# oriolfornes/ExplaiNN

Hardware: AMD Instinct MI355X
Metric: sequences/sec (fwd+bwd), 200bp one-hot, 300 units, batch 1024 (higher is better)
Workload: dtype f32

## Files before the change

explainn_amd/csrc/api.hip:

```cpp
#include <stdarg.h>
#include <stdio.h>
#include <string.h>

#include <cstdlib>
#include <cstring>

#include "common.h"

static thread_local char g_err[512] = "";

void explainn_set_error(const char* fmt, ...) {
    va_list ap;
    va_start(ap, fmt);
    vsnprintf(g_err, sizeof(g_err), fmt, ap);
    va_end(ap);
}

extern "C" const char* explainn_last_error(void) { return g_err; }

namespace {
struct Carver {
    int64_t off = 0;
    char* base = nullptr;
    template <typename T>
    void take(T** p, int64_t count) {
        off = (off + 255) & ~int64_t(255);
        if (base) *p = reinterpret_cast<T*>(base + off);
        off += count * (int64_t)sizeof(T);
    }
};

void carve(explainn_ctx* c, Carver& cv) {
    const int64_t U = c->U, U4 = c->U4, n = c->n, Bs = c->Bs, NS = c->NS, K4 = c->K4;
    cv.take(&c->codesT, (int64_t)c->L * Bs);
    cv.take(&c->pk2, (int64_t)c->PW * Bs);
    cv.take(&c->nmask, (int64_t)c->NW * Bs);
    cv.take(&c->bm, (int64_t)4 * (Bs / 64) * c->Lp);
    cv.take(&c->G, K4 * K4);
    cv.take(&c->m, K4);
    cv.take(&c->alpha, U4);
    cv.take(&c->shift, U4);
    cv.take(&c->mug, U4);
    cv.take(&c->sig1, U4);
    cv.take(&c->Gw, U4 * K4);
    cv.take(&c->Wt, (int64_t)c->Uq * c->k * 20);
    cv.take(&c->Wf, (int64_t)conv_tiles_padded(c->U, c->k) * conv_ksteps(c->k) * 3 * 512);
    cv.take(&c->Wsg, (int64_t)conv_tiles_padded(c->U, c->k) * 32);
    const int64_t Upad = (int64_t)32 * conv_tiles_padded(c->U, c->k);
    cv.take(&c->ext, Upad * n * Bs + 64);
    cv.take(&c->idx, Upad * n * Bs + 64);
    cv.take(&c->qs0, U * NS);
    cv.take(&c->qS1p, U * c->QCH * NS);
    cv.take(&c->qS2p, U * c->QCH * NS * NS);
    cv.take(&c->qbar, U * NS);
    cv.take(&c->VC, U * FC_H * NS);
    cv.take(&c->A2, U * FC_H * NS);
    cv.take(&c->A2f, c->NQ <= FC_BF_MAXN ? 0 : U * FC_MT * fc_nk4q(c->NQ) * 256);
    cv.take(&c->A2h, c->NQ <= FC_BF_MAXN ? U * FC_MT * fc_ks32(c->NQ) * 3 * 256 : 0);
    cv.take(&c->sh2, U * FC_H);
    cv.take(&c->sig2, U * FC_H);
    cv.take(&c->z, U * Bs);
    cv.take(&c->zhat, U * Bs);
    cv.take(&c->o, U * Bs);
    cv.take(&c->sig3, U);
    c->ZBLK = fc_fwd_blocks((int)Bs, c->NQ);
    cv.take(&c->z12p, U * c->ZBLK * 2);
    cv.take(&c->bits, U * Bs + 4);
    cv.take(&c->dz, U * Bs + 4);
    cv.take(&c->EQp, U * c->ACH * FC_H * NS);
    cv.take(&c->Sep, U * c->ACH * FC_H);
    cv.take(&c->EQs, U * FC_H * NS);
    cv.take(&c->Ttf, U * fc_nw16(c->NQ) * 3 * 4 * 256);
    cv.take(&c->Mff, U * fc_nw16(c->NQ) * 4 * fc_nw16(c->NQ) * 64);
    cv.take(&c->k0p, U * NS);
    cv.take(&c->dy, U4 * n * Bs);
    cv.take(&c->S12p, U * fc_ng(c->NQ) * (Bs / 16) * 2);
    cv.take(&c->Dspp, U * (Bs / 4) * K4);
    cv.take(&c->dlogits, (int64_t)c->maxB * c->T);
    cv.take(&c->flags, 64);
    cv.take(&c->dlT, (int64_t)c->T * Bs);
    cv.take(&c->gWp, c->T > HEAD_GEMM_MIN_T ? (int64_t)head_gw_chunks(c->maxB) * c->T * (c->U + 1) : 0);
    cv.take(&c->lossp, 256);
    cv.take(&c->site_cnt, U4 * Bs);
    cv.take(&c->site_off, U4 * Bs);
    cv.off = (cv.off + 255) & ~int64_t(255);
}

int check_batch(const explainn_ctx* c, int B) {
    if (!c) { explainn_set_error("null context"); return EXPLAINN_E_ARG; }
    if (B < 1 || B > c->maxB) {
        explainn_set_error("batch %d outside [1, max_batch=%d]", B, c->maxB);
        return EXPLAINN_E_ARG;
    }
    return EXPLAINN_OK;
}

#define TRY(call)                    \
    do {                             \
        int rc_ = (call);            \
        if (rc_ != EXPLAINN_OK) return rc_; \
    } while (0)

const char* const kStageNames[ST_COUNT] = {
    "pack_tables", "moments", "prep1_stats", "conv_pool", "qmom", "prep2", "fc_fwd", "head_fwd",
    "loss", "head_bwd", "passA", "mid", "passB", "conv_bwd", "fin_bwd"};
#define STAGE(id, call)                                                                 \
    do {                                                                                \
        if (c->timing) HIP_TRY(hipEventRecord(c->ev0[id], s));                          \
        TRY(call);                                                                      \
        if (c->timing) { HIP_TRY(hipEventRecord(c->ev1[id], s)); c->timed |= 1u << (id); } \
    } while (0)

int eval_front(explainn_ctx* c, const float* x, int B, const explainn_params* p, hipStream_t s) {
    c->fwd_B = 0; c->tail_B = 0;
    if (c->dense) {
        if (!x) { explainn_set_error("dense input mode needs x"); return EXPLAINN_E_ARG; }
        c->staged_B = 0;
    } else {
        TRY(launch_pack(c, x, B, false, s));
    }
    if (!(c->eval_valid && p->version != 0 && p->version == c->eval_version)) {
        TRY(launch_prep1_tables(c, p, s));
        TRY(launch_prep1(c, p, B, false, s));
        TRY(launch_prep2(c, p, B, false, s));
        c->eval_valid = true;
        c->eval_version = p->version;
// ... 408 lines not shown
```

explainn_amd/csrc/bwd.hip:

```cpp
#include "common.h"

typedef float f32x16b __attribute__((ext_vector_type(16)));
typedef float f32x2 __attribute__((ext_vector_type(2)));
typedef float f32x4b __attribute__((ext_vector_type(4)));

__global__ __launch_bounds__(1024) void mid_fused_kernel(
    const float* __restrict__ EQp, const float* __restrict__ Sep, const float* __restrict__ A2,
    const float* __restrict__ sh2, const float* __restrict__ sig2, const float* __restrict__ fc1_w,
    const float* __restrict__ fc2_w, const float* __restrict__ g2, const double* __restrict__ qbar,
    const float* __restrict__ VC, float* __restrict__ Ttf,
    float* __restrict__ Mff, float* __restrict__ k0p, float* __restrict__ g_fc2_w, float* __restrict__ g_bn2_w,
    float* __restrict__ g_bn2_b, float* __restrict__ g_fc1_b, float* __restrict__ g_fc1_w, int n,
    int NS, int NW16, int B, int ACH, float scale) {
    extern __shared__ float fsm[];
    const int ld = n + 1;
    float* V1s = fsm;
    float* A2s = V1s + FC_H * ld;
    float* EQl = A2s + FC_H * ld;
    float* Ms = EQl + FC_H * ld;
    float* qb = Ms + n * n;
    float* se = qb + n;
    float* md2s = se + FC_H;
    float* cfs = md2s + FC_H;
    float* md2hs = cfs + FC_H;
    float* VCl = md2hs + FC_H;
    float* svl = VCl + FC_H * ld;
    float* gsl = svl + FC_H;
    float* sgl = gsl + FC_H;
    const int u = blockIdx.x, tid = threadIdx.x;
    STAMP(0);
    {
        constexpr int NPASS = 3;
        for (int e0 = tid; e0 < FC_H * n; e0 += 1024 * NPASS) {
            float v1[NPASS], a2[NPASS], vc[NPASS];
            int dst[NPASS];
#pragma unroll
            for (int it = 0; it < NPASS; ++it) {
                const int e = e0 + 1024 * it;
                const bool on = e < FC_H * n;
                const int ec = on ? e : 0, r = ec / n, w = ec - r * n;
                const uint32_t ch = (uint32_t)(u * FC_H + r);
                dst[it] = on ? r * ld + w : -1;
                v1[it] = fc1_w[(size_t)ch * n + w];
                a2[it] = A2[(size_t)ch * NS + w];
                vc[it] = VC[(size_t)ch * NS + w];
            }
#pragma unroll
            for (int it = 0; it < NPASS; ++it) { KEEP(v1[it]); KEEP(a2[it]); KEEP(vc[it]); }
#pragma unroll
            for (int it = 0; it < NPASS; ++it)
                if (dst[it] >= 0) { V1s[dst[it]] = v1[it]; A2s[dst[it]] = a2[it]; VCl[dst[it]] = vc[it]; }
        }
    }
    for (int e0 = tid; e0 < FC_H * n; e0 += 1024 * 3) {
        double eq[3] = {0, 0, 0};
        for (int c0 = 0; c0 < ACH; c0 += 4) {
            float pv[3][4];
#pragma unroll
            for (int it = 0; it < 3; ++it) {
                const int e = e0 + 1024 * it, ec = e < FC_H * n ? e : 0;
                const int w = ec / FC_H, r = ec % FC_H;
#pragma unroll
                for (int i = 0; i < 4; ++i)
                    pv[it][i] = EQp[(((size_t)u * ACH + min(c0 + i, ACH - 1)) * NS + w) * FC_H + r];
// ... 31 lines not shown
    __syncthreads();
    STAMP(1);
    const double sc = (double)scale;
    if (tid < FC_H) {
        const int r = tid;
        const size_t ch = (size_t)u * FC_H + r;
        double sAE = 0, sVE = 0;
        const double ser = (double)se[r];
        for (int w = 0; w < n; ++w) {
            const double eq = (double)EQl[r * ld + w];
            sAE = fma((double)A2s[r * ld + w], eq, sAE);
            sVE = fma((double)V1s[r * ld + w], eq - ser * qbd[w], sVE);
        }
        const double v2 = (double)fc2_w[ch], sg = (double)sig2[ch];
        g_fc2_w[ch] = (float)(sc * (sAE + (double)sh2[ch] * ser));
        const double db2 = sc * v2 * ser, dg2 = sc * v2 / sg * sVE;
        g_bn2_b[ch] = (float)db2;
        g_bn2_w[ch] = (float)dg2;
        g_fc1_b[ch] = 0.f;
        md2s[r] = (float)(db2 / (double)B);
        md2hs[r] = (float)(dg2 / (double)B);
        cfs[r] = (float)((dg2 / (double)B) / sg);
        svl[r] = (float)v2; gsl[r] = (float)((double)g2[ch] / sg); sgl[r] = (float)((double)B / sg);
    }
    __syncthreads();
    STAMP(2);
    const int NT2 = NW16;
    const int ntile_m = NT2 * NT2;
    {
        const int wave = tid >> 6, lane = tid & 63, c = lane & 15, gq = lane >> 4;
        for (int tile = wave; tile < ntile_m; tile += 16) {
            const int vt = tile / NT2, wt = tile % NT2;
            const int va = 16 * vt + c, wb = 16 * wt + c;
            const bool alive = va < n, blive = wb < n;
            const float* acol = V1s + min(va, n - 1);
            const float* bcol = A2s + min(wb, n - 1);
            f32x4b acc = f32x4b{0.f, 0.f, 0.f, 0.f};
#pragma unroll
            for (int q0 = 0; q0 < FC_H / 4; q0 += 5) {
                float av[5], bv[5];
#pragma unroll
                for (int q = 0; q < 5; ++q) {
                    const int r = 4 * (q0 + q) + gq;
                    av[q] = cfs[r] * acol[r * ld];
                    bv[q] = bcol[r * ld];
                }
#pragma unroll
                for (int q = 0; q < 5; ++q)
                    acc = __builtin_amdgcn_mfma_f32_16x16x4f32(alive ? av[q] : 0.f, blive ? bv[q] : 0.f, acc, 0, 0, 0);
            }
#pragma unroll
            for (int i = 0; i < 4; ++i) {
                const int v = 16 * vt + 4 * gq + i;
                Mff[(((size_t)u * NW16 + wt) * (4 * NW16) + 4 * vt + i) * 64 + 16 * gq + c] = acc[i];
                if (v < n && wb < n) Ms[v * n + wb] = acc[i];
            }
        }
    }
    STAMP(3);
    const int busy = min(ntile_m, 8) * 64;
    for (int e = tid - busy; e < FC_H * NS; e += 1024 - busy) {
        if (e < 0) break;
        const int r = e / NS, w = e % NS;
        const size_t ch = (size_t)u * FC_H + r;
        const double sv = sc * (double)svl[r];
        float tv = 0.f;
        if (w < n) {
            tv = (float)(sv * (double)A2s[r * ld + w]);
            const double hq = (double)VCl[r * ld + w] * (double)sgl[r];
            const double val = (double)gsl[r] *
                               (sv * (double)EQl[r * ld + w] -
                                (double)md2s[r] * (double)B * qbd[w] -
                                (double)md2hs[r] * hq);
            g_fc1_w[ch * n + w] = (float)val;
        }
        {
            const uint32_t hb = __float_as_uint(tv) & 0xffff0000u;
            const float r1 = tv - __uint_as_float(hb);
            const uint32_t mb = __float_as_uint(r1) & 0xffff0000u;
            const float r2 = r1 - __uint_as_float(mb);
            uint16_t* tb = reinterpret_cast<uint16_t*>(Ttf) + ((size_t)u * NW16 + (w >> 4)) * (3 * 4 * 512) +
                           ((size_t)(r >> 5) * 64 + 16 * ((r >> 3) & 3) + (w & 15)) * 8 + (r & 7);
            tb[0] = (uint16_t)(hb >> 16);
            tb[4 * 512] = (uint16_t)(mb >> 16);
            tb[8 * 512] = (uint16_t)(__float_as_uint(r2) >> 16);
        }
    }
    __syncthreads();
    STAMP(4);
    for (int w = tid; w < NS; w += 1024) {
        double k0 = 0;
        if (w < n) {
            for (int r = 0; r < FC_H; ++r) k0 = fma((double)A2s[r * ld + w], (double)md2s[r], k0);
            for (int v = 0; v < n; ++v) k0 -= qbd[v] * (double)Ms[v * n + w];
        }
        k0p[(size_t)u * NS + w] = (float)k0;
    }
    STAMP(5);
}

__global__ __launch_bounds__(1024) void mid_big_kernel(
    const float* __restrict__ EQp, const float* __restrict__ Sep, const float* __restrict__ A2,
    const float* __restrict__ sh2, const float* __restrict__ sig2, const float* __restrict__ fc1_w,
    const float* __restrict__ fc2_w, const float* __restrict__ g2, const double* __restrict__ qbar,
    const float* __restrict__ VC, float* __restrict__ EQs,
    float* __restrict__ Ttf, float* __restrict__ Mff,
    float* __restrict__ k0p, float* __restrict__ g_fc2_w, float* __restrict__ g_bn2_w,
    float* __restrict__ g_bn2_b, float* __restrict__ g_fc1_b, float* __restrict__ g_fc1_w, int n,
    int NS, int NW16, int B, int ACH, float scale) {
    extern __shared__ float bsm[];
    const int ld = n + 1;
    float* V1s = bsm;
    float* A2s = V1s + FC_H * ld;
    float* qb = A2s + FC_H * ld;
    float* se = qb + n;
    float* md2s = se + FC_H;
    float* cfs = md2s + FC_H;
    float* md2hs = cfs + FC_H;
    float* kco = md2hs + FC_H;
    const int u = blockIdx.x, tid = threadIdx.x;
    constexpr int NT = 1024;
    for (int e = tid; e < FC_H * n; e += NT) {
        const int r = e / n, w = e % n;
        const size_t ch = (size_t)u * FC_H + r;
        V1s[r * ld + w] = fc1_w[ch * n + w];
        A2s[r * ld + w] = A2[ch * NS + w];
    }
    for (int e = tid; e < FC_H * n; e += NT) {
        const int w = e / FC_H, r = e % FC_H;
        const size_t ch = (size_t)u * FC_H + r;
        double eq = 0;
        for (int c0 = 0; c0 < ACH; c0 += 8) {
            float pv[8];
#pragma unroll
            for (int i = 0; i < 8; ++i)
                pv[i] = EQp[(((size_t)u * ACH + min(c0 + i, ACH - 1)) * NS + w) * FC_H + r];
#pragma unroll
            for (int i = 0; i < 8; ++i) KEEP(pv[i]);
#pragma unroll
            for (int i = 0; i < 8; ++i) eq += (c0 + i < ACH) ? (double)pv[i] : 0.0;
        }
        EQs[ch * NS + w] = (float)eq;
    }
    for (int w = tid; w < n; w += NT) qb[w] = (float)qbar[(size_t)u * NS + w];
    for (int r = tid; r < FC_H; r += NT) {
        double s = 0;
        for (int c = 0; c < ACH; ++c) s += (double)Sep[((size_t)u * ACH + c) * FC_H + r];
        se[r] = (float)s;
    }
    __syncthreads();
    const double sc = (double)scale;
    {
        const int r = tid >> 3, part = tid & 7;
        const int rr = r < FC_H ? r : FC_H - 1;
        const size_t ch = (size_t)u * FC_H + rr;
        double sAE = 0, sVE = 0, qv = 0;
        const double ser = (double)se[rr];
        for (int w = part; w < n; w += 8) {
            const double eq = (double)EQs[ch * NS + w];
            const double qw = qbar[(size_t)u * NS + w];
            sAE = fma((double)A2s[rr * ld + w], eq, sAE);
            sVE = fma((double)V1s[rr * ld + w], eq - ser * qw, sVE);
            qv = fma((double)V1s[rr * ld + w], qw, qv);
        }
#pragma unroll
        for (int off = 1; off < 8; off <<= 1) {
            sAE += __shfl_xor(sAE, off, 64); sVE += __shfl_xor(sVE, off, 64); qv += __shfl_xor(qv, off, 64);
        }
        if (r < FC_H && part == 0) {
            const double v2 = (double)fc2_w[ch], sg = (double)sig2[ch];
            g_fc2_w[ch] = (float)(sc * (sAE + (double)sh2[ch] * ser));
            const double db2 = sc * v2 * ser, dg2 = sc * v2 / sg * sVE;
            g_bn2_b[ch] = (float)db2;
            g_bn2_w[ch] = (float)dg2;
            g_fc1_b[ch] = 0.f;
            md2s[r] = (float)(db2 / (double)B);
            md2hs[r] = (float)(dg2 / (double)B);
            const double cf = (dg2 / (double)B) / sg;
            cfs[r] = (float)cf;
            kco[r] = (float)(db2 / (double)B - cf * qv);
        }
    }
    __syncthreads();
    {
        const int wave = tid >> 6, lane = tid & 63, rc = lane & 31, kk = lane >> 5;
        const int NT2 = (NS + 31) >> 5;
        for (int tile = wave; tile < NT2 * NT2; tile += NT / 64) {
            const int vt = tile / NT2, wt = tile % NT2;
            const int va = 32 * vt + rc, wb = 32 * wt + rc;
            const bool alive = va < n, blive = wb < n;
            const float* acol = V1s + min(va, n - 1);
            const float* bcol = A2s + min(wb, n - 1);
            f32x16b acc;
#pragma unroll
            for (int g = 0; g < 16; ++g) acc[g] = 0.f;
#pragma unroll 5
            for (int s2 = 0; s2 < FC_H / 2; ++s2) {
                const int r = 2 * s2 + kk;
                const float a = alive ? cfs[r] * acol[r * ld] : 0.f;
                const float bb = blive ? bcol[r * ld] : 0.f;
                acc = __builtin_amdgcn_mfma_f32_32x32x2f32(a, bb, acc, 0, 0, 0);
            }
            if (wb < NS) {
#pragma unroll
                for (int g = 0; g < 16; ++g) {
                    const int v = 32 * vt + (g & 3) + 8 * (g >> 2) + 4 * kk;
                    if (v < NS) {
                        if (v < 16 * NW16 && wb < 16 * NW16)
                            Mff[(((size_t)u * NW16 + (wb >> 4)) * (4 * NW16) + 4 * (v >> 4) + (v & 3)) * 64 +
                                16 * ((v >> 2) & 3) + (wb & 15)] = acc[g];
                    }
                }
            }
        }
    }
    for (int e = tid; e < FC_H * NS; e += NT) {
        const int r = e / NS, w = e % NS;
        const size_t ch = (size_t)u * FC_H + r;
        const double sv = sc * (double)fc2_w[ch];
        float tv = 0.f;
        if (w < n) {
            tv = (float)(sv * (double)A2s[r * ld + w]);
            const double sg = (double)sig2[ch];
            const double hq = (double)VC[ch * NS + w] * (double)B / sg;
            const double val = ((double)g2[ch] / sg) *
                               (sv * (double)EQs[ch * NS + w] -
                                (double)md2s[r] * (double)B * qbar[(size_t)u * NS + w] -
                                (double)md2hs[r] * hq);
            g_fc1_w[ch * n + w] = (float)val;
        }
        {
            const uint32_t hb = __float_as_uint(tv) & 0xffff0000u;
            const float r1 = tv - __uint_as_float(hb);
            const uint32_t mb = __float_as_uint(r1) & 0xffff0000u;
            const float r2 = r1 - __uint_as_float(mb);
            uint16_t* tb = reinterpret_cast<uint16_t*>(Ttf) + ((size_t)u * NW16 + (w >> 4)) * (3 * 4 * 512) +
                           ((size_t)(r >> 5) * 64 + 16 * ((r >> 3) & 3) + (w & 15)) * 8 + (r & 7);
            tb[0] = (uint16_t)(hb >> 16);
            tb[4 * 512] = (uint16_t)(mb >> 16);
            tb[8 * 512] = (uint16_t)(__float_as_uint(r2) >> 16);
        }
    }
    for (int w = tid; w < NS; w += NT) {
        double k0 = 0;
        if (w < n)
            for (int r = 0; r < FC_H; ++r) k0 = fma((double)A2s[r * ld + w], (double)kco[r], k0);
        k0p[(size_t)u * NS + w] = (float)k0;
    }
}

static size_t mid_big_lds(int n) {
    return ((size_t)2 * FC_H * (n + 1) + n + 5 * FC_H) * sizeof(float);
}

static size_t mid_fused_lds(int n) {
    return ((size_t)4 * FC_H * (n + 1) + (size_t)n * n + n + 7 * FC_H + 2) * sizeof(float) + (size_t)n * sizeof(double);
}

int launch_mid_bwd(explainn_ctx* c, const explainn_params* p, const explainn_grads* g, int B,
                   hipStream_t s) {
    if (c->n <= 72) {
        hipLaunchKernelGGL(mid_fused_kernel, dim3(c->U), dim3(1024), mid_fused_lds(c->n), s, c->EQp,
                           c->Sep, c->A2, c->sh2, c->sig2, p->fc1_w, p->fc2_w, p->bn2_w, c->qbar,
                           c->VC, c->Ttf, c->Mff, c->k0p, g->fc2_w, g->bn2_w, g->bn2_b,
                           g->fc1_b, g->fc1_w, c->n, c->NS, fc_nw16(c->NQ), B, c->ACH,
                           c->fwd_scale);
        LAUNCH_CHECK();
        return EXPLAINN_OK;
    }
    hipLaunchKernelGGL(mid_big_kernel, dim3(c->U), dim3(1024), mid_big_lds(c->n), s, c->EQp, c->Sep,
                       c->A2, c->sh2, c->sig2, p->fc1_w, p->fc2_w, p->bn2_w, c->qbar, c->VC, c->EQs,
                       c->Ttf, c->Mff, c->k0p, g->fc2_w, g->bn2_w, g->bn2_b, g->fc1_b,
                       g->fc1_w, c->n, c->NS, fc_nw16(c->NQ), B, c->ACH,
                       c->fwd_scale);
    LAUNCH_CHECK();
    return EXPLAINN_OK;
}

#define FIN_THREADS 320
#define FIN_MAXGRP 8
struct fin_args {
    const float* S12p; const double* m; const double* Gw; const double* mug; const double* sig1;
    const float* g1; float* g_conv_w; float* g_conv_b; float* g_bn1_w; float* g_bn1_b;
    int K4; int freeze_n; int NG;
    int dsp_stride, dsp_count;
};

__device__ __forceinline__ void fin_unit(const fin_args& f, const float* __restrict__ Dspp, int u,
                                         int tid, int nthr, int Bs, int B) {
    const int K4 = f.K4;
    const int NT = f.dsp_stride, nt = f.dsp_count;
    const int NT16 = Bs / 16, nt16 = (B + 15) / 16;
    __shared__ double fin_red[2][16];
    double S1 = 0, S2 = 0;
    for (int t = tid; t < f.NG * nt16; t += nthr) {
        const int grp = t / nt16, tl = t - grp * nt16;
        const float2 pv = *reinterpret_cast<const float2*>(&f.S12p[(((size_t)u * f.NG + grp) * NT16 + tl) * 2]);
        S1 += (double)pv.x; S2 += (double)pv.y;
    }
    S1 = wave_sum_d(S1); S2 = wave_sum_d(S2);
    if ((tid & 63) == 0) { fin_red[0][tid >> 6] = S1; fin_red[1][tid >> 6] = S2; }
    __syncthreads();
    S1 = 0; S2 = 0;
    for (int w = 0; w < (nthr + 63) / 64; ++w) { S1 += fin_red[0][w]; S2 += fin_red[1][w]; }
    const double sg = f.sig1[u], a = (double)f.g1[u] / sg, mu = f.mug[u];
    __shared__ double fin_part[FIN_MAXGRP][4 * MAX_K];
    const int ngrp = min(FIN_MAXGRP, max(1, nthr / K4));
    const int grp = tid / K4, i = tid - grp * K4;
    if (grp < ngrp) {
        double D = 0;
        for (int t0 = grp; t0 < nt; t0 += 16 * ngrp) {
            float pv[16];
#pragma unroll
            for (int q = 0; q < 16; ++q) pv[q] = Dspp[((size_t)u * NT + min(t0 + q * ngrp, nt - 1)) * K4 + i];
#pragma unroll
            for (int q = 0; q < 16; ++q) KEEP(pv[q]);
#pragma unroll
            for (int q = 0; q < 16; ++q) D += (t0 + q * ngrp < nt) ? (double)pv[q] : 0.0;
        }
        fin_part[grp][i] = D;
    }
    __syncthreads();
    if (tid < K4) {
        double D = 0;
        for (int q = 0; q < ngrp; ++q) D += fin_part[q][tid];
// ... 288 lines not shown
```

explainn_amd/csrc/common.h:

```cpp
#pragma once
#include <hip/hip_runtime.h>
#include <stdint.h>

#include "../../include/explainn_hip.h"

#define FC_H 100
#define HEAD_RB 8
#define HEAD_GEMM_MIN_T 8
#define HEAD_GW_MAXCH 32
__host__ inline int head_gw_chunks(int B) { int c = (B + 127) / 128; return c < 1 ? 1 : (c > HEAD_GW_MAXCH ? HEAD_GW_MAXCH : c); }
#define POOLW 7
#define BN_EPS_D 1e-5
#define BN_MOM_D 0.1
#define WAVE 64
#define MAX_K 32
#define MAX_NQ 160

struct explainn_ctx {
    int U, k, L, T, maxB, device;
    int Lo, n;
    int U4, Uq;
    int NQ, NS;
    int Bs;
    int K4;
    int QCH;
    int ACH;
    bool timing; unsigned timed;
    hipEvent_t ev0[16], ev1[16];
    int fwd_B;
    int tail_B;
    int fwd_drop;
    float fwd_scale;
    char* base; int64_t bytes;
    uint8_t* codesT;
    uint32_t* pk2;
    uint32_t* nmask;
    int PW, NW;
    unsigned long long* bm;
    int Lp;
    double* G;
    double* m;
    float* alpha;
    float* shift;
    double* mug;
    double* sig1;
    double* Gw;
    float* Wt;
    uint32_t* Wsg;
    uint16_t* Wf;
    float* ext;
    uint8_t* idx;
    float* qs0;
    float* qS1p;
    float* qS2p;
    double* qbar;
    float* VC;
    float* A2;
    float* A2f;
    float* A2h;
    float* sh2;
    float* sig2;
    float* z;
    float* zhat;
    float* o;
    float* sig3;
    double* z12p;
    int ZBLK;
    uint4* bits;
    float* dz;
    float* EQp;
    float* Sep;
    float* EQs;
    float* Ttf;
    float* Mff;
    float* k0p;
    float* dy;
    float* S12p;
    float* Dspp;
    int dsp_stride, dsp_count;
    float* dlogits;
    float* dlT;
    int loss_blocks, loss_n; float* loss_out;
    float* gWp;
    double* lossp;
    int staged_B;
    bool eval_valid;
    uint64_t eval_version;
    bool dense;
    const float* dense_x;
    int* flags;
    int* site_cnt;
    int* site_off;
};

enum explainn_stage {
    ST_PACK, ST_MOMENTS, ST_PREP1, ST_CONV_POOL, ST_QMOM, ST_PREP2, ST_FC_FWD, ST_HEAD_FWD, ST_LOSS,
    ST_HEAD_BWD, ST_PASSA, ST_MID, ST_PASSB, ST_CONV_BWD, ST_FIN, ST_COUNT
};

void explainn_set_error(const char* fmt, ...);
#define HIP_TRY(expr)                                                              \
    do {                                                                           \
        hipError_t e_ = (expr);                                                    \
        if (e_ != hipSuccess) {                                                    \
            explainn_set_error("%s failed: %s (%s:%d)", #expr, hipGetErrorString(e_), \
                               __FILE__, __LINE__);                                \
            return EXPLAINN_E_HIP;                                                 \
        }                                                                          \
    } while (0)
#define LAUNCH_CHECK()  HIP_TRY(hipGetLastError())

int launch_pack(explainn_ctx* c, const float* x, int B, bool counts, hipStream_t s);
int launch_prep1(explainn_ctx* c, const explainn_params* p, int B, bool train, hipStream_t s);
int launch_moments(explainn_ctx* c, int B, hipStream_t s);
int launch_prep1_tables(explainn_ctx* c, const explainn_params* p, hipStream_t s);
int launch_conv_pool(explainn_ctx* c, const explainn_params* p, int B, bool want_idx, hipStream_t s);
int launch_pack_tables(explainn_ctx* c, const float* x, const explainn_params* p, int B, hipStream_t s);
int launch_pack_codes(explainn_ctx* c, const uint8_t* codes, int B, int rc, hipStream_t s);
int launch_conv_act(explainn_ctx* c, int B, float* acts, hipStream_t s);
int launch_filter_act_max(explainn_ctx* c, int B, const uint8_t* select, float* umax, hipStream_t s);
int launch_filter_sites(explainn_ctx* c, int B, const uint8_t* select, const float* thr, int cap,
                        int* site_total, int* pfm, uint8_t* hit, hipStream_t s);
int launch_qmoments(explainn_ctx* c, int B, hipStream_t s);
int launch_prep2(explainn_ctx* c, const explainn_params* p, int B, bool train, hipStream_t s);
int launch_fc_fwd(explainn_ctx* c, const explainn_params* p, int B, bool train,
                  const uint8_t* keep_mask, float drop_p, uint64_t seed, hipStream_t s);
int launch_head_fwd(explainn_ctx* c, const explainn_params* p, int B, bool train, float* logits,
// ... 105 lines not shown
    return u < U;
}
__host__ inline int units_grid(int U) { return (U + 7) & ~7; }

__device__ __forceinline__ float qval(float alpha, float ext, float shift) {
    return __expf(fmaf(alpha, ext, shift));
}

__device__ __forceinline__ float wave_sum(float v) {
#pragma unroll
    for (int off = 32; off > 0; off >>= 1) v += __shfl_xor(v, off, 64);
    return v;
}
__device__ __forceinline__ double wave_sum_d(double v) {
#pragma unroll
    for (int off = 32; off > 0; off >>= 1) v += __shfl_xor(v, off, 64);
    return v;
}

__host__ __device__ constexpr int chunk_count(int len) { return (len + 35) / 36; }
__host__ __device__ constexpr int chunk_len(int len) {
    return (((len + chunk_count(len) - 1) / chunk_count(len)) + 3) & ~3;
}
__host__ __device__ constexpr int ns_stride(int NQ) { return chunk_count(NQ) * chunk_len(NQ); }

static inline int nq_bucket(int n) {
    static const int b[] = {4, 8, 12, 16, 20, 24, 26, 28, 32, 40, 48, 56, 64, 72, 84, 96,
                            112, 128, 140, 160};
    for (unsigned i = 0; i < sizeof(b) / sizeof(b[0]); ++i)
        if (b[i] >= n) return b[i];
    return 0;
}
__host__ __device__ constexpr int nq_lower(int NQ) {
    constexpr int b[] = {0, 4, 8, 12, 16, 20, 24, 26, 28, 32, 40, 48, 56, 64, 72, 84, 96, 112, 128, 140, 160};
    int lo = 0;
    for (int i = 1; i < 21; ++i) if (b[i] == NQ) lo = b[i - 1];
    return lo;
}
#define FC_MT 7
__host__ __device__ constexpr int fc_nk4(int NQ) { return (NQ + 3) / 4; }
__host__ __device__ constexpr int fc_nk4q(int NQ) { return (fc_nk4(NQ) + 3) / 4; }
__host__ __device__ constexpr int fc_nw16(int NQ) { return (NQ + 15) / 16; }
#ifndef FC_BTW
#define FC_BTW 4
#endif
__host__ __device__ constexpr int fc_fwd_waves(int NQ) { return 4; }
__host__ __device__ constexpr int fc_fwd_blocks(int B, int NQ) {
    return ((B + 15) / 16 + fc_fwd_waves(NQ) * FC_BTW - 1) / (fc_fwd_waves(NQ) * FC_BTW);
}
#define FC_BF_MAXN 96
__host__ __device__ constexpr int fc_ks32(int NQ) { return (NQ + 31) / 32; }
__host__ __device__ constexpr int fc_wgt(int NQ) { return fc_nw16(NQ) <= 2 ? fc_nw16(NQ) : 3; }
__host__ __device__ constexpr int fc_ng(int NQ) { return (fc_nw16(NQ) + fc_wgt(NQ) - 1) / fc_wgt(NQ); }

#define NQ_DISPATCH(NQv, CALL)                                                        \
    switch (NQv) {                                                                    \
        case 4: { CALL(4); } break;     case 8: { CALL(8); } break;                   \
        case 12: { CALL(12); } break;   case 16: { CALL(16); } break;                 \
        case 20: { CALL(20); } break;   case 24: { CALL(24); } break;                 \
        case 26: { CALL(26); } break;   case 28: { CALL(28); } break;                 \
        case 32: { CALL(32); } break;   case 40: { CALL(40); } break;                 \
        case 48: { CALL(48); } break;   case 56: { CALL(56); } break;                 \
        case 64: { CALL(64); } break;   case 72: { CALL(72); } break;                 \
        case 84: { CALL(84); } break;   case 96: { CALL(96); } break;                 \
        case 112: { CALL(112); } break; case 128: { CALL(128); } break;               \
        case 140: { CALL(140); } break; case 160: { CALL(160); } break;               \
        default: explainn_set_error("pooled length bucket %d not instantiated", NQv); \
                 return EXPLAINN_E_UNSUPPORTED;                                       \
    }
```

explainn_amd/csrc/fc.hip:

```cpp
#include "common.h"

typedef float f32x4 __attribute__((ext_vector_type(4)));
#define MFMA16(a, b, c) __builtin_amdgcn_mfma_f32_16x16x4f32((a), (b), (c), 0, 0, 0)

__device__ __forceinline__ uint32_t mix32(uint32_t x) {
    x ^= x >> 16; x *= 0x7feb352dU; x ^= x >> 15; x *= 0x846ca68bU; x ^= x >> 16;
    return x;
}

__device__ __forceinline__ void fmac_under_mask(float& acc, float a, float b, unsigned long long m) {
    unsigned long long saved;
    asm volatile("s_and_saveexec_b64 %0, %4\n\tv_fmac_f32 %1, %2, %3\n\ts_mov_b64 exec, %0"
                 : "=&s"(saved), "+v"(acc) : "v"(a), "v"(b), "s"(m) : "scc");
}
__device__ __forceinline__ uint32_t shift_in_bit(uint32_t nib, unsigned long long m) {
    unsigned long long cout;
    asm volatile("v_addc_co_u32_e64 %0, %1, %0, %0, %2" : "+v"(nib), "=s"(cout) : "s"(m));
    return nib;
}

template <int MODE>
__device__ __forceinline__ void fc_epilogue_tile(const f32x4& acc, int t, int g, const float* v2s,
                                                 uint32_t& rs, uint32_t thresh16, const uint8_t* km,
                                                 float& zp, uint32_t (&words)[4]) {
// ... 630 lines not shown
        if (wave == 1) {
#pragma unroll
            for (int t = 0; t < FC_MT; ++t)
#pragma unroll
                for (int j = 0; j < WGT; ++j)
                    red[(t * WGT + j) * 64 + lane] = make_float4(acc[t][j][0], acc[t][j][1], acc[t][j][2], acc[t][j][3]);
        }
        __syncthreads();
        if (wave != 0) return;
#pragma unroll
        for (int t = 0; t < FC_MT; ++t)
#pragma unroll
            for (int j = 0; j < WGT; ++j) {
                const float4 v = red[(t * WGT + j) * 64 + lane];
                acc[t][j][0] += v.x; acc[t][j][1] += v.y; acc[t][j][2] += v.z; acc[t][j][3] += v.w;
                if ((t * WGT + j) % 4 == 3) __builtin_amdgcn_sched_barrier(0);
            }
    }
#pragma unroll
    for (int j = 0; j < WGT; ++j) {
        const int w = w0 + 16 * j + c;
#pragma unroll
        for (int t = 0; t < FC_MT; ++t) {
            const int r = 16 * t + 4 * g;
            if (r < FC_H) {
                const float4 v = make_float4(acc[t][j][0], acc[t][j][1], acc[t][j][2], acc[t][j][3]);
                if (w == n) *reinterpret_cast<float4*>(&Sep[((size_t)u * ACH + ch) * FC_H + r]) = v;
                else if (w < NS) *reinterpret_cast<float4*>(&EQp[(((size_t)u * ACH + ch) * NS + w) * FC_H + r]) = v;
            }
        }
    }
    STAMP(3);
}

int launch_passA(explainn_ctx* c, int B, const pa_head_args* head, hipStream_t s) {
    pa_head_args h = {};
    if (head) h = *head;
#define CALL(N)                                                                                  \
    if (h.mode)                                                                                  \
        hipLaunchKernelGGL((passA_kernel<N, true>), dim3(c->ACH, c->U, pa_ng(N)), dim3(64 * PA_WAVES), 0, s, \
                           c->ext, c->alpha, c->shift, c->dz, c->bits, c->EQp, c->Sep, c->n, c->Bs, \
                           B, c->ACH, h, c->U);                                                  \
    else                                                                                         \
        hipLaunchKernelGGL((passA_kernel<N, false>), dim3(c->ACH, c->U, pa_ng(N)), dim3(64 * PA_WAVES), 0, s, \
                           c->ext, c->alpha, c->shift, c->dz, c->bits, c->EQp, c->Sep, c->n, c->Bs, \
                           B, c->ACH, h, c->U)
    NQ_DISPATCH(c->NQ, CALL);
#undef CALL
    LAUNCH_CHECK();
    return EXPLAINN_OK;
}

template <int NQ>
__global__ __launch_bounds__(256, 2) void passB_kernel(
    const float* __restrict__ ext, const float* __restrict__ alpha,
    const float* __restrict__ shift, const float* __restrict__ dz, const uint4* __restrict__ bits,
    const float* __restrict__ Ttf, const float* __restrict__ Mff, const float* __restrict__ k0p,
    const double* __restrict__ mug, const double* __restrict__ sig1, float* __restrict__ dy,
    float* __restrict__ S12p, int n, int Bs, int B, int U) {
    constexpr int NS = ns_stride(NQ), NW16 = fc_nw16(NQ), WGT = fc_wgt(NQ), NG = fc_ng(NQ);
    constexpr int TBW = 3 * 4 * 256, MK = 4 * NW16;
    extern __shared__ __attribute__((aligned(16))) float smemB[];
    float* Tf = smemB;
    float* Mf = Tf + WGT * TBW;
    float* k0s = Mf + WGT * MK * 64;
    int u, bx;
    if (!unit_chunk_of_block(U, u, bx)) return;
    const int grp = blockIdx.z, tid = threadIdx.x, lane = tid & 63, wave = tid >> 6;
    const int c = lane & 15, g = lane >> 4;
    const int j0 = grp * WGT;
    const int ntile = min(WGT, NW16 - j0);
    STAMP(0);
    {
        constexpr int NT4 = WGT * TBW / 4, NM4 = WGT * MK * 16, N4 = NT4 + NM4;
        const float4* srcT = reinterpret_cast<const float4*>(Ttf + ((size_t)u * NW16 + j0) * TBW);
        const float4* srcM = reinterpret_cast<const float4*>(Mff + ((size_t)u * NW16 + j0) * MK * 64);
        const int lim_t = ntile * TBW / 4, lim_m = ntile * MK * 16;
        float4* dst = reinterpret_cast<float4*>(Tf);
        float4 tv[(N4 + 255) / 256];
#pragma unroll
        for (int i = 0; i < (N4 + 255) / 256; ++i) {
            const int e = tid + i * 256;
            float4 v = make_float4(0.f, 0.f, 0.f, 0.f);
            if (e < NT4) { if (e < lim_t) v = srcT[e]; }
            else if (e < N4) { if (e - NT4 < lim_m) v = srcM[e - NT4]; }
            tv[i] = v;
        }
#pragma unroll
        for (int i = 0; i < (N4 + 255) / 256; ++i)
            if (tid + i * 256 < N4) dst[tid + i * 256] = tv[i];
    }
    for (int i = tid; i < WGT * 16; i += 256) {
        const int w = 16 * j0 + i;
        k0s[i] = (w < NS) ? k0p[(size_t)u * NS + w] : 0.f;
    }
    __syncthreads();
    STAMP(1);
    const float* __restrict__ eu = ext + (size_t)u * n * Bs;
    float* __restrict__ dyu = dy + (size_t)u * n * Bs;
    const float a1 = alpha[u], s1 = shift[u];
    const float mu = (float)mug[u];
    const float isg = (float)(1.0 / sig1[u]);
    for (int it = 0; it < PB_BTW; ++it) {
        const int bt = (bx * 4 + wave) * PB_BTW + it;
        if (bt * 16 >= B) break;
        const int b = bt * 16 + c;
        const bool live = b < B;
        const int bc = min(b, Bs - 1);
        float exr[MK];
#pragma unroll
        for (int kq = 0; kq < MK; ++kq) exr[kq] = eu[min(16 * (kq >> 2) + 4 * g + (kq & 3), n - 1) * Bs + bc];
        const uint4 wv = bits[(size_t)u * Bs + bc];
        const float dzb = dz[(size_t)u * Bs + bc];
#pragma unroll
        for (int kq = 0; kq < MK; ++kq) KEEP(exr[kq]);
        float nq[MK];
#pragma unroll
        for (int kq = 0; kq < MK; ++kq)
            nq[kq] = (16 * (kq >> 2) + 4 * g + (kq & 3) < n) ? -qval(a1, exr[kq], s1) : 0.f;
        float sA = 0.f, sB = 0.f;
        if (it == 0) STAMP_AFTER_LOADS(2);
        f32x4 accP[WGT];
#pragma unroll
        for (int j = 0; j < WGT; ++j) accP[j] = f32x4{0.f, 0.f, 0.f, 0.f};
        const uint32_t wsv[4] = {wv.x, wv.y, wv.z, wv.w};
#pragma unroll
        for (int kk = 0; kk < 4; ++kk) {
            const uint32_t wg = wsv[kk] >> (8 * g);
            u32x4 bv;
#pragma unroll
            for (int i = 0; i < 4; ++i) {
                const int m0 = __builtin_amdgcn_sbfe(wg, 2 * i, 1), m1 = __builtin_amdgcn_sbfe(wg, 2 * i + 1, 1);
                bv[i] = ((uint32_t)m0 & 0x00003f80u) | ((uint32_t)m1 & 0x3f800000u);
            }
            const bf16x8 bfr = __builtin_bit_cast(bf16x8, bv);
#pragma unroll
            for (int j = 0; j < WGT; ++j)
#pragma unroll
                for (int p3 = 0; p3 < 3; ++p3) {
                    const bf16x8 afr = *reinterpret_cast<const bf16x8*>(
                        reinterpret_cast<const uint16_t*>(Tf) + (((j * 3 + p3) * 4 + kk) * 64 + lane) * 8);
                    accP[j] = __builtin_amdgcn_mfma_f32_16x16x32_bf16(afr, bfr, accP[j], 0, 0, 0);
                }
        }
        f32x4 acc[WGT];
#pragma unroll
        for (int j = 0; j < WGT; ++j) {
            const float4 v = *reinterpret_cast<const float4*>(&k0s[16 * j + 4 * g]);
            acc[j][0] = -v.x; acc[j][1] = -v.y; acc[j][2] = -v.z; acc[j][3] = -v.w;
        }
#pragma unroll
        for (int kq = 0; kq < MK; ++kq)
#pragma unroll
            for (int j = 0; j < WGT; ++j) acc[j] = MFMA16(Mf[(j * MK + kq) * 64 + lane], nq[kq], acc[j]);
#pragma unroll
        for (int j = 0; j < WGT; ++j)
#pragma unroll
            for (int i = 0; i < 4; ++i) acc[j][i] = fmaf(dzb, accP[j][i], acc[j][i]);
        if (it == 0) STAMP(3);
#pragma unroll
        for (int j = 0; j < WGT; ++j) {
            if (j >= ntile) break;
#pragma unroll
            for (int i = 0; i < 4; ++i) {
                float nqv = 0.f, ex = 0.f;
#pragma unroll
                for (int gg = 0; gg < NG; ++gg) {
                    const int kq = 4 * (gg * WGT + j) + i;
                    if (kq < MK && gg == grp) { nqv = nq[kq]; ex = exr[kq]; }
                }
                const int w = 16 * (j0 + j) + 4 * g + i;
                const float dyv = (live && w < n) ? -acc[j][i] * nqv : 0.f;
                sA += dyv;
                sB = fmaf(dyv, (ex - mu) * isg, sB);
                if (w < n && b < Bs) dyu[w * Bs + b] = dyv;
            }
        }
        if (it == 0) STAMP(4);
        sA = wave_sum(sA);
        sB = wave_sum(sB);
        if (lane == 0) {
            float* d = S12p + (((size_t)u * NG + grp) * (Bs / 16) + bt) * 2;
            d[0] = sA; d[1] = sB;
        }
    }
    STAMP(5);
}

template <int NQ>
static size_t passB_lds() {
    constexpr int WGT = fc_wgt(NQ), MK = 4 * fc_nw16(NQ);
    return (size_t)(WGT * 3 * 4 * 256 + WGT * MK * 64 + WGT * 16) * sizeof(float);
}

int launch_passB(explainn_ctx* c, int B, hipStream_t s) {
    const int tiles = (B + 15) / 16;
    const int nx = (tiles + 4 * PB_BTW - 1) / (4 * PB_BTW);
#define CALL(N)                                                                                  \
    hipLaunchKernelGGL(passB_kernel<N>, dim3(nx, units_grid(c->U), fc_ng(N)), dim3(256), passB_lds<N>(), s,  \
                       c->ext, c->alpha, c->shift, c->dz, c->bits, c->Ttf, c->Mff, c->k0p, c->mug,  \
                       c->sig1, c->dy, c->S12p, c->n, c->Bs, B, c->U)
    NQ_DISPATCH(c->NQ, CALL);
#undef CALL
    LAUNCH_CHECK();
    return EXPLAINN_OK;
}

int fc_configure(explainn_ctx* c) {
#define CALL(N)                                                                              \
    if (passB_lds<N>() > 48 * 1024)                                                          \
        HIP_TRY(hipFuncSetAttribute(reinterpret_cast<const void*>(&passB_kernel<N>),          \
                                    hipFuncAttributeMaxDynamicSharedMemorySize,              \
                                    (int)passB_lds<N>()));                                   \
    { int rc;                                                                                \
      if ((rc = fc_fwd_configure_nm<N, 0>()) || (rc = fc_fwd_configure_nm<N, 1>()) ||        \
          (rc = fc_fwd_configure_nm<N, 2>()) || (rc = fc_fwd_configure_nm<N, 3>())) return rc; }
    NQ_DISPATCH(c->NQ, CALL);
#undef CALL
    return EXPLAINN_OK;
}
```

Baseline: 5.084 million.

## Replace fp32 MFMA M-product in passB with split-bf16 MFMA and prefetch inputs

The M matrix is now stored as three bf16 pieces (hi/mid/lo split) in a new Mtf layout, so passB computes M·nq with 16x16x32 bf16 MFMAs (9 piece products) instead of the fp32 16x16x4 MFMA. It also software-pipelines the per-tile global loads (ext, bits, dz) one iteration ahead, precomputes per-group selections, simplifies the bit-to-bf16 expansion, and raises occupancy for small NW16 via launch bounds. The mid kernels write the new split layout. The risk is extra conversion ALU work and register pressure, plus a small precision difference from the 3-piece bf16 split.

```diff
diff --git a/explainn_amd/csrc/api.hip b/explainn_amd/csrc/api.hip
--- a/explainn_amd/csrc/api.hip
+++ b/explainn_amd/csrc/api.hip
@@ -71,7 +71,7 @@
     cv.take(&c->Sep, U * c->ACH * FC_H);
     cv.take(&c->EQs, U * FC_H * NS);
     cv.take(&c->Ttf, U * fc_nw16(c->NQ) * 3 * 4 * 256);
-    cv.take(&c->Mff, U * fc_nw16(c->NQ) * 4 * fc_nw16(c->NQ) * 64);
+    cv.take(&c->Mtf, U * fc_nw16(c->NQ) * fc_mks(c->NQ) * 3 * 256);
     cv.take(&c->k0p, U * NS);
     cv.take(&c->dy, U4 * n * Bs);
     cv.take(&c->S12p, U * fc_ng(c->NQ) * (Bs / 16) * 2);
diff --git a/explainn_amd/csrc/bwd.hip b/explainn_amd/csrc/bwd.hip
--- a/explainn_amd/csrc/bwd.hip
+++ b/explainn_amd/csrc/bwd.hip
@@ -9,7 +9,7 @@
     const float* __restrict__ sh2, const float* __restrict__ sig2, const float* __restrict__ fc1_w,
     const float* __restrict__ fc2_w, const float* __restrict__ g2, const double* __restrict__ qbar,
     const float* __restrict__ VC, float* __restrict__ Ttf,
-    float* __restrict__ Mff, float* __restrict__ k0p, float* __restrict__ g_fc2_w, float* __restrict__ g_bn2_w,
+    float* __restrict__ Mtf, float* __restrict__ k0p, float* __restrict__ g_fc2_w, float* __restrict__ g_bn2_w,
     float* __restrict__ g_bn2_b, float* __restrict__ g_fc1_b, float* __restrict__ g_fc1_w, int n,
     int NS, int NW16, int B, int ACH, float scale) {
     extern __shared__ float fsm[];
@@ -147,7 +147,6 @@
 #pragma unroll
             for (int i = 0; i < 4; ++i) {
                 const int v = 16 * vt + 4 * gq + i;
-                Mff[(((size_t)u * NW16 + wt) * (4 * NW16) + 4 * vt + i) * 64 + 16 * gq + c] = acc[i];
                 if (v < n && wb < n) Ms[v * n + wb] = acc[i];
             }
         }
@@ -191,6 +190,14 @@
         }
         k0p[(size_t)u * NS + w] = (float)k0;
     }
+    for (int e = tid - NS; e < 4 * NW16 * 16 * NW16; e += 1024) {
+        if (e < 0) continue;
+        const int v0 = 4 * (e / (16 * NW16)), w = e % (16 * NW16);
+        float mv[4];
+#pragma unroll
+        for (int i = 0; i < 4; ++i) mv[i] = (v0 + i < n && w < n) ? Ms[(v0 + i) * n + w] : 0.f;
+        m_pieces_store4(Mtf, u, NW16, v0, w, mv);
+    }
     STAMP(5);
 }
 
@@ -199,7 +206,7 @@
     const float* __restrict__ sh2, const float* __restrict__ sig2, const float* __restrict__ fc1_w,
     const float* __restrict__ fc2_w, const float* __restrict__ g2, const double* __restrict__ qbar,
     const float* __restrict__ VC, float* __restrict__ EQs,
-    float* __restrict__ Ttf, float* __restrict__ Mff,
+    float* __restrict__ Ttf, float* __restrict__ Mtf,
     float* __restrict__ k0p, float* __restrict__ g_fc2_w, float* __restrict__ g_bn2_w,
     float* __restrict__ g_bn2_b, float* __restrict__ g_fc1_b, float* __restrict__ g_fc1_w, int n,
     int NS, int NW16, int B, int ACH, float scale) {
@@ -296,14 +303,15 @@
                 const float bb = blive ? bcol[r * ld] : 0.f;
                 acc = __builtin_amdgcn_mfma_f32_32x32x2f32(a, bb, acc, 0, 0, 0);
             }
-            if (wb < NS) {
-#pragma unroll
-                for (int g = 0; g < 16; ++g) {
-                    const int v = 32 * vt + (g & 3) + 8 * (g >> 2) + 4 * kk;
-                    if (v < NS) {
-                        if (v < 16 * NW16 && wb < 16 * NW16)
-                            Mff[(((size_t)u * NW16 + (wb >> 4)) * (4 * NW16) + 4 * (v >> 4) + (v & 3)) * 64 +
-                                16 * ((v >> 2) & 3) + (wb & 15)] = acc[g];
+            if (wb < NS && wb < 16 * NW16) {
+#pragma unroll
+                for (int h = 0; h < 4; ++h) {
+                    const int v0 = 32 * vt + 8 * h + 4 * kk;
+                    const float mv[4] = {acc[4 * h], acc[4 * h + 1], acc[4 * h + 2], acc[4 * h + 3]};
+                    if (v0 < NS && v0 < 16 * NW16) {
+                        if (NW16 <= 6) m_pieces_store4(Mtf, u, NW16, v0, wb, mv);
+                        else
+                            for (int i = 0; i < 4; ++i) Mtf[m_fp32_index(u, NW16, v0 + i, wb)] = mv[i];
                     }
                 }
             }
@@ -357,7 +365,7 @@
     if (c->n <= 72) {
         hipLaunchKernelGGL(mid_fused_kernel, dim3(c->U), dim3(1024), mid_fused_lds(c->n), s, c->EQp,
                            c->Sep, c->A2, c->sh2, c->sig2, p->fc1_w, p->fc2_w, p->bn2_w, c->qbar,
-                           c->VC, c->Ttf, c->Mff, c->k0p, g->fc2_w, g->bn2_w, g->bn2_b,
+                           c->VC, c->Ttf, c->Mtf, c->k0p, g->fc2_w, g->bn2_w, g->bn2_b,
                            g->fc1_b, g->fc1_w, c->n, c->NS, fc_nw16(c->NQ), B, c->ACH,
                            c->fwd_scale);
         LAUNCH_CHECK();
@@ -365,7 +373,7 @@
     }
     hipLaunchKernelGGL(mid_big_kernel, dim3(c->U), dim3(1024), mid_big_lds(c->n), s, c->EQp, c->Sep,
                        c->A2, c->sh2, c->sig2, p->fc1_w, p->fc2_w, p->bn2_w, c->qbar, c->VC, c->EQs,
-                       c->Ttf, c->Mff, c->k0p, g->fc2_w, g->bn2_w, g->bn2_b, g->fc1_b,
+                       c->Ttf, c->Mtf, c->k0p, g->fc2_w, g->bn2_w, g->bn2_b, g->fc1_b,
                        g->fc1_w, c->n, c->NS, fc_nw16(c->NQ), B, c->ACH,
                        c->fwd_scale);
     LAUNCH_CHECK();
diff --git a/explainn_amd/csrc/common.h b/explainn_amd/csrc/common.h
--- a/explainn_amd/csrc/common.h
+++ b/explainn_amd/csrc/common.h
@@ -72,7 +72,7 @@
     float* Sep;
     float* EQs;
     float* Ttf;
-    float* Mff;
+    float* Mtf;
     float* k0p;
     float* dy;
     float* S12p;
@@ -284,6 +284,35 @@
 __host__ __device__ constexpr int fc_ks32(int NQ) { return (NQ + 31) / 32; }
 __host__ __device__ constexpr int fc_wgt(int NQ) { return fc_nw16(NQ) <= 2 ? fc_nw16(NQ) : 3; }
 __host__ __device__ constexpr int fc_ng(int NQ) { return (fc_nw16(NQ) + fc_wgt(NQ) - 1) / fc_wgt(NQ); }
+__host__ __device__ constexpr bool fc_mbf(int NQ) { return fc_nw16(NQ) <= 6; }
+__host__ __device__ constexpr int fc_mks(int NQ) { return (fc_nw16(NQ) + 1) / 2; }
+__device__ __forceinline__ size_t m_fp32_index(size_t u, int NW16, int v, int w) {
+    return ((u * NW16 + (w >> 4)) * (4 * NW16) + 4 * (v >> 4) + (v & 3)) * 64 + 16 * ((v >> 2) & 3) + (w & 15);
+}
+__device__ __forceinline__ void m_pieces_store4(float* Mtf, size_t u, int NW16, int v0, int w, const float x[4]) {
+    const int mks = (NW16 + 1) >> 1;
+    uint32_t p[3][2];
+#pragma unroll
+    for (int h = 0; h < 2; ++h) {
+        uint32_t pc[3][2];
+#pragma unroll
+        for (int e = 0; e < 2; ++e) {
+            const float xv = x[2 * h + e];
+            const uint32_t hb = __float_as_uint(xv) & 0xffff0000u;
+            const float r1 = xv - __uint_as_float(hb);
+            const uint32_t mb = __float_as_uint(r1) & 0xffff0000u;
+            const float r2 = r1 - __uint_as_float(mb);
+            pc[0][e] = hb >> 16; pc[1][e] = mb >> 16; pc[2][e] = __float_as_uint(r2) >> 16;
+        }
+#pragma unroll
+        for (int q = 0; q < 3; ++q) p[q][h] = pc[q][0] | (pc[q][1] << 16);
+    }
+    uint16_t* base = reinterpret_cast<uint16_t*>(Mtf) +
+                     ((((u * NW16 + (w >> 4)) * mks + (v0 >> 5)) * 3) * 64 + 16 * ((v0 >> 2) & 3) + (w & 15)) * 8 +
+                     4 * ((v0 >> 4) & 1);
+#pragma unroll
+    for (int q = 0; q < 3; ++q) *reinterpret_cast<uint2*>(base + q * 512) = make_uint2(p[q][0], p[q][1]);
+}
 
 #define NQ_DISPATCH(NQv, CALL)                                                        \
     switch (NQv) {                                                                    \
diff --git a/explainn_amd/csrc/fc.hip b/explainn_amd/csrc/fc.hip
--- a/explainn_amd/csrc/fc.hip
+++ b/explainn_amd/csrc/fc.hip
@@ -706,18 +706,22 @@
 }
 
 template <int NQ>
-__global__ __launch_bounds__(256, 2) void passB_kernel(
+__global__ __launch_bounds__(256, fc_nw16(NQ) <= 2 ? 5 : 2) void passB_kernel(
     const float* __restrict__ ext, const float* __restrict__ alpha,
     const float* __restrict__ shift, const float* __restrict__ dz, const uint4* __restrict__ bits,
-    const float* __restrict__ Ttf, const float* __restrict__ Mff, const float* __restrict__ k0p,
+    const float* __restrict__ Ttf, const float* __restrict__ Mtf, const float* __restrict__ k0p,
     const double* __restrict__ mug, const double* __restrict__ sig1, float* __restrict__ dy,
     float* __restrict__ S12p, int n, int Bs, int B, int U) {
     constexpr int NS = ns_stride(NQ), NW16 = fc_nw16(NQ), WGT = fc_wgt(NQ), NG = fc_ng(NQ);
-    constexpr int TBW = 3 * 4 * 256, MK = 4 * NW16;
+    constexpr bool MBF = fc_mbf(NQ);
+    constexpr int MKS = fc_mks(NQ);
+    constexpr int TBW = 3 * 4 * 256;
+    constexpr int MBW = MBF ? MKS * 3 * 256 : 4 * NW16 * 64;
+    constexpr int MK = 4 * NW16, MKP = 8 * MKS;
     extern __shared__ __attribute__((aligned(16))) float smemB[];
     float* Tf = smemB;
     float* Mf = Tf + WGT * TBW;
-    float* k0s = Mf + WGT * MK * 64;
+    float* k0s = Mf + WGT * MBW;
     int u, bx;
     if (!unit_chunk_of_block(U, u, bx)) return;
     const int grp = blockIdx.z, tid = threadIdx.x, lane = tid & 63, wave = tid >> 6;
@@ -726,10 +730,10 @@
     const int ntile = min(WGT, NW16 - j0);
     STAMP(0);
     {
-        constexpr int NT4 = WGT * TBW / 4, NM4 = WGT * MK * 16, N4 = NT4 + NM4;
+        constexpr int NT4 = WGT * TBW / 4, NM4 = WGT * MBW / 4, N4 = NT4 + NM4;
         const float4* srcT = reinterpret_cast<const float4*>(Ttf + ((size_t)u * NW16 + j0) * TBW);
-        const float4* srcM = reinterpret_cast<const float4*>(Mff + ((size_t)u * NW16 + j0) * MK * 64);
-        const int lim_t = ntile * TBW / 4, lim_m = ntile * MK * 16;
+        const float4* srcM = reinterpret_cast<const float4*>(Mtf + ((size_t)u * NW16 + j0) * MBW);
+        const int lim_t = ntile * TBW / 4, lim_m = ntile * MBW / 4;
         float4* dst = reinterpret_cast<float4*>(Tf);
         float4 tv[(N4 + 255) / 256];
 #pragma unroll
@@ -755,79 +759,149 @@
     const float a1 = alpha[u], s1 = shift[u];
     const float mu = (float)mug[u];
     const float isg = (float)(1.0 / sig1[u]);
+    const uint4* __restrict__ bu = bits + (size_t)u * Bs;
+    const float* __restrict__ dzu = dz + (size_t)u * Bs;
+    const int bt0 = (bx * 4 + wave) * PB_BTW;
+    float exr[MK], dzb = 0.f;
+    uint4 wv = make_uint4(0u, 0u, 0u, 0u);
+    auto issue = [&](int bt) {
+        const int bc = min(bt * 16 + c, Bs - 1);
+        const char* __restrict__ eb = reinterpret_cast<const char*>(eu);
+        const uint32_t boff = (uint32_t)bc * 4u;
+        uint32_t rstride = (uint32_t)Bs * 4u;
+        int g4 = 4 * g;
+        asm volatile("" : "+v"(rstride), "+v"(g4));
+#pragma unroll
+        for (int kq = 0; kq < MK; ++kq)
+            exr[kq] = *reinterpret_cast<const float*>(
+                eb + (__umul24(rstride, (uint32_t)min(16 * (kq >> 2) + g4 + (kq & 3), n - 1)) + boff));
+        wv = *reinterpret_cast<const uint4*>(reinterpret_cast<const char*>(bu) + (uint32_t)bc * 16u);
+        dzb = *reinterpret_cast<const float*>(reinterpret_cast<const char*>(dzu) + boff);
+    };
+    if (bt0 * 16 < B) issue(bt0);
+#pragma unroll 1
     for (int it = 0; it < PB_BTW; ++it) {
-        const int bt = (bx * 4 + wave) * PB_BTW + it;
+        const int bt = bt0 + it;
         if (bt * 16 >= B) break;
         const int b = bt * 16 + c;
         const bool live = b < B;
-        const int bc = min(b, Bs - 1);
-        float exr[MK];
-#pragma unroll
-        for (int kq = 0; kq < MK; ++kq) exr[kq] = eu[min(16 * (kq >> 2) + 4 * g + (kq & 3), n - 1) * Bs + bc];
-        const uint4 wv = bits[(size_t)u * Bs + bc];
-        const float dzb = dz[(size_t)u * Bs + bc];
-#pragma unroll
-        for (int kq = 0; kq < MK; ++kq) KEEP(exr[kq]);
-        float nq[MK];
-#pragma unroll
-        for (int kq = 0; kq < MK; ++kq)
-            nq[kq] = (16 * (kq >> 2) + 4 * g + (kq & 3) < n) ? -qval(a1, exr[kq], s1) : 0.f;
-        float sA = 0.f, sB = 0.f;
-        if (it == 0) STAMP_AFTER_LOADS(2);
+        float ex[MK];
+#pragma unroll
+        for (int kq = 0; kq < MK; ++kq) ex[kq] = exr[kq];
+        const uint32_t wsv[4] = {wv.x, wv.y, wv.z, wv.w};
+        const float dzc = dzb;
+        float nq[MKP];
+        int gq4 = 4 * g;
+        asm volatile("" : "+v"(gq4));
+#pragma unroll
+        for (int kq = 0; kq < MKP; ++kq)
+            nq[kq] = (kq < MK && 16 * (kq >> 2) + gq4 + (kq & 3) < n) ? -qval(a1, ex[kq], s1) : 0.f;
+        float nqs[WGT][4], exs[WGT][4];
+#pragma unroll
+        for (int j = 0; j < WGT; ++j)
+#pragma unroll
+            for (int i = 0; i < 4; ++i) {
+                float nqv = 0.f, exv = 0.f;
+#pragma unroll
+                for (int gg = 0; gg < NG; ++gg) {
+                    const int kq = 4 * (gg * WGT + j) + i;
+                    if (kq < MK && gg == grp) { nqv = nq[kq]; exv = ex[kq]; }
+                }
+                nqs[j][i] = nqv; exs[j][i] = exv;
+            }
+        if (it == 0) STAMP(2);
+        if (it + 1 < PB_BTW && (bt + 1) * 16 < B) issue(bt + 1);
+        __builtin_amdgcn_sched_barrier(0);
+        uint32_t foff = (uint32_t)lane * 8u;
+        asm volatile("" : "+v"(foff));
+        const uint16_t* Tb = reinterpret_cast<const uint16_t*>(Tf) + foff;
+        const uint16_t* Mb = reinterpret_cast<const uint16_t*>(Mf) + foff;
         f32x4 accP[WGT];
 #pragma unroll
         for (int j = 0; j < WGT; ++j) accP[j] = f32x4{0.f, 0.f, 0.f, 0.f};
-        const uint32_t wsv[4] = {wv.x, wv.y, wv.z, wv.w};
 #pragma unroll
         for (int kk = 0; kk < 4; ++kk) {
-            const uint32_t wg = wsv[kk] >> (8 * g);
             u32x4 bv;
 #pragma unroll
             for (int i = 0; i < 4; ++i) {
-                const int m0 = __builtin_amdgcn_sbfe(wg, 2 * i, 1), m1 = __builtin_amdgcn_sbfe(wg, 2 * i + 1, 1);
-                bv[i] = ((uint32_t)m0 & 0x00003f80u) | ((uint32_t)m1 & 0x3f800000u);
+                const uint32_t sh = (uint32_t)(8 * g + 2 * i);
+                const uint32_t two = __builtin_amdgcn_ubfe(wsv[kk], sh, 1u) |
+                                     (__builtin_amdgcn_ubfe(wsv[kk], sh + 1u, 1u) << 16);
+                bv[i] = __umul24(two, 0x3f80u);
             }
             const bf16x8 bfr = __builtin_bit_cast(bf16x8, bv);
 #pragma unroll
             for (int j = 0; j < WGT; ++j)
 #pragma unroll
                 for (int p3 = 0; p3 < 3; ++p3) {
-                    const bf16x8 afr = *reinterpret_cast<const bf16x8*>(
-                        reinterpret_cast<const uint16_t*>(Tf) + (((j * 3 + p3) * 4 + kk) * 64 + lane) * 8);
+                    const bf16x8 afr = *reinterpret_cast<const bf16x8*>(Tb + ((j * 3 + p3) * 4 + kk) * 512);
                     accP[j] = __builtin_amdgcn_mfma_f32_16x16x32_bf16(afr, bfr, accP[j], 0, 0, 0);
                 }
+            __builtin_amdgcn_sched_barrier(0);
         }
         f32x4 acc[WGT];
 #pragma unroll
         for (int j = 0; j < WGT; ++j) {
             const float4 v = *reinterpret_cast<const float4*>(&k0s[16 * j + 4 * g]);
-            acc[j][0] = -v.x; acc[j][1] = -v.y; acc[j][2] = -v.z; acc[j][3] = -v.w;
-        }
-#pragma unroll
-        for (int kq = 0; kq < MK; ++kq)
-#pragma unroll
-            for (int j = 0; j < WGT; ++j) acc[j] = MFMA16(Mf[(j * MK + kq) * 64 + lane], nq[kq], acc[j]);
-#pragma unroll
-        for (int j = 0; j < WGT; ++j)
-#pragma unroll
-            for (int i = 0; i < 4; ++i) acc[j][i] = fmaf(dzb, accP[j][i], acc[j][i]);
+            acc[j][0] = fmaf(dzc, accP[j][0], -v.x); acc[j][1] = fmaf(dzc, accP[j][1], -v.y);
+            acc[j][2] = fmaf(dzc, accP[j][2], -v.z); acc[j][3] = fmaf(dzc, accP[j][3], -v.w);
+        }
+        if constexpr (MBF) {
+#pragma unroll
+            for (int s = 0; s < MKS; ++s) {
+                u32x4 qp[3];
+#pragma unroll
+                for (int i = 0; i < 4; ++i) {
+                    uint32_t pc[3][2];
+#pragma unroll
+                    for (int e = 0; e < 2; ++e) {
+                        const float x = nq[8 * s + 2 * i + e];
+                        const uint32_t hb = __float_as_uint(x) & 0xffff0000u;
+                        const float r1 = x - __uint_as_float(hb);
+                        const uint32_t mb = __float_as_uint(r1) & 0xffff0000u;
+                        const float r2 = r1 - __uint_as_float(mb);
+                        pc[0][e] = hb >> 16; pc[1][e] = mb >> 16; pc[2][e] = __float_as_uint(r2) >> 16;
+                    }
+#pragma unroll
+                    for (int p3 = 0; p3 < 3; ++p3) qp[p3][i] = pc[p3][0] | (pc[p3][1] << 16);
+                }
+#pragma unroll
+                for (int j = 0; j < WGT; ++j)
+#pragma unroll
+                    for (int pa = 0; pa < 3; ++pa) {
+                        const bf16x8 afr = *reinterpret_cast<const bf16x8*>(Mb + ((j * MKS + s) * 3 + pa) * 512);
+#pragma unroll
+                        for (int pb = 0; pb < 3; ++pb)
+                            acc[j] = __builtin_amdgcn_mfma_f32_16x16x32_bf16(afr, __builtin_bit_cast(bf16x8, qp[pb]),
+                                                                             acc[j], 0, 0, 0);
+                    }
+                __builtin_amdgcn_sched_barrier(0);
+            }
+        } else {
+            const float* Mq = Mf + (foff >> 3);
+#pragma unroll
+            for (int kq = 0; kq < MK; ++kq)
+#pragma unroll
+                for (int j = 0; j < WGT; ++j) acc[j] = MFMA16(Mq[(j * MK + kq) * 64], nq[kq], acc[j]);
+        }
         if (it == 0) STAMP(3);
+        float sA = 0.f, sB = 0.f;
+        char* __restrict__ db = reinterpret_cast<char*>(dyu);
+        const uint32_t dboff = (uint32_t)b * 4u;
+        uint32_t dstride = (uint32_t)Bs * 4u;
+        int g4 = 4 * g;
+        asm volatile("" : "+v"(dstride), "+v"(g4));
 #pragma unroll
         for (int j = 0; j < WGT; ++j) {
             if (j >= ntile) break;
 #pragma unroll
             for (int i = 0; i < 4; ++i) {
-                float nqv = 0.f, ex = 0.f;
-#pragma unroll
-                for (int gg = 0; gg < NG; ++gg) {
-                    const int kq = 4 * (gg * WGT + j) + i;
-                    if (kq < MK && gg == grp) { nqv = nq[kq]; ex = exr[kq]; }
-                }
-                const int w = 16 * (j0 + j) + 4 * g + i;
+                const float nqv = nqs[j][i], exv = exs[j][i];
+                const int w = 16 * (j0 + j) + g4 + i;
                 const float dyv = (live && w < n) ? -acc[j][i] * nqv : 0.f;
                 sA += dyv;
-                sB = fmaf(dyv, (ex - mu) * isg, sB);
-                if (w < n && b < Bs) dyu[w * Bs + b] = dyv;
+                sB = fmaf(dyv, (exv - mu) * isg, sB);
+                if (w < n && b < Bs) *reinterpret_cast<float*>(db + (__umul24(dstride, (uint32_t)w) + dboff)) = dyv;
             }
         }
         if (it == 0) STAMP(4);
@@ -843,8 +917,8 @@
 
 template <int NQ>
 static size_t passB_lds() {
-    constexpr int WGT = fc_wgt(NQ), MK = 4 * fc_nw16(NQ);
-    return (size_t)(WGT * 3 * 4 * 256 + WGT * MK * 64 + WGT * 16) * sizeof(float);
+    constexpr int WGT = fc_wgt(NQ), MBW = fc_mbf(NQ) ? fc_mks(NQ) * 3 * 256 : 4 * fc_nw16(NQ) * 64;
+    return (size_t)(WGT * 3 * 4 * 256 + WGT * MBW + WGT * 16) * sizeof(float);
 }
 
 int launch_passB(explainn_ctx* c, int B, hipStream_t s) {
@@ -852,7 +926,7 @@
     const int nx = (tiles + 4 * PB_BTW - 1) / (4 * PB_BTW);
 #define CALL(N)                                                                                  \
     hipLaunchKernelGGL(passB_kernel<N>, dim3(nx, units_grid(c->U), fc_ng(N)), dim3(256), passB_lds<N>(), s,  \
-                       c->ext, c->alpha, c->shift, c->dz, c->bits, c->Ttf, c->Mff, c->k0p, c->mug,  \
+                       c->ext, c->alpha, c->shift, c->dz, c->bits, c->Ttf, c->Mtf, c->k0p, c->mug,  \
                        c->sig1, c->dy, c->S12p, c->n, c->Bs, B, c->U)
     NQ_DISPATCH(c->NQ, CALL);
 #undef CALL
```

After: 5.114 million, median of 6. Within noise of the previous version (+0.6%).
